# solufast-cvprojects/multigriddet

Hardware: NVIDIA B200
Metric: encode+decode/NMS images/sec, COCO 608×608, 1–8 B200; % HBM peak (higher is better)
Workload: dtype f32

## Files before the change

multigriddet_b200/csrc/api.cu:

```cuda
#include <math.h>
#include <stdarg.h>
#include <stdio.h>
#include <string.h>

#include <chrono>
#include <functional>
#include <mutex>
#include <string>
#include <thread>
#include <vector>

#include "common.cuh"
#include "dlpack_abi.h"

namespace {

thread_local std::string t_error;

int fail(int code, const char* fmt, ...)
{
    char buf[512];
    va_list ap;
    va_start(ap, fmt);
    vsnprintf(buf, sizeof(buf), fmt, ap);
// ... 286 lines not shown

int env_chunk(const char* name)
{
    const char* e = getenv(name);
    return e ? atoi(e) : 0;
}

int chunk_images(const HeadGeom& g, int batch)
{
    long long n = (32ll << 20) / ((long long)g.cells * 4);
    if (const int e = env_chunk("MGD_ENCODE_CHUNK_IMAGES")) n = e;
    if (n < 1) n = 1;
    if (n > batch) n = batch;
    return (int)n;
}

int decode_chunk_images(const HeadGeom& g, int batch)
{
    long long n = (1ll << 30) / ((long long)g.cells * (long long)sizeof(Cand));
    if (const int e = env_chunk("MGD_DECODE_CHUNK_IMAGES")) n = e;
    if (n < 1) n = 1;
    if (n > batch) n = batch;
    return (int)n;
}

struct DeferredStatus {
    int* word[64] = {};
    ~DeferredStatus()
    {
        for (int d = 0; d < 64; ++d) if (word[d]) cudaFree(word[d]);
        cudaGetLastError();
    }
};
thread_local DeferredStatus t_deferred;

int deferred_status_word(int device, int** out)
{
    if (!t_deferred.word[device]) {
        CUDA_TRY(cudaMalloc(reinterpret_cast<void**>(&t_deferred.word[device]), 256));
        CUDA_TRY(cudaMemset(t_deferred.word[device], 0, 256));
    }
    *out = t_deferred.word[device];
    return MGD_OK;
}

int status_to_error(int st)
{
    if (st & 1) return fail(MGD_ERR_CLASS_RANGE, "class id must be less than num_classes");
    if (st & 2)
        return fail(MGD_ERR_INVALID_ARGUMENT,
                    "negative class id on a valid box (the reference would write a wrong channel)");
    return MGD_OK;
}

struct EncodeScratch { int* table; BoxRec* recs; };

bool step_pdl()
{
    static int v = -1;
    if (v < 0) { const char* e = getenv("MGD_STEP_PDL"); v = e ? atoi(e) : 1; }
    return v != 0;
}

int encode_assign_all(const HeadGeom& g, const float* boxes, int batch, int N, float* const* y,
                      cudaStream_t stream, int* d_status, int tf_compat, std::vector<EncodeArgs>* chunks)
{
    nvtx_range nv("mgd:encode assign (preprocess_true_boxes)");
    const Alloc al{nullptr, stream};
    const int step = chunk_images(g, batch);
    for (int b0 = 0; b0 < batch; b0 += step) {
        const int nb = batch - b0 < step ? batch - b0 : step;
        EncodeArgs a;
        a.g = g;
        a.B = nb;
        a.N = N;
        a.boxes = boxes + (size_t)b0 * N * 5;
        for (int l = 0; l < g.L; ++l)
            a.y[l] = y[l] + (size_t)b0 * g.gh[l] * g.gw[l] * g.D[l];
        a.tf_compat = tf_compat;
        a.status = d_status;
        a.stats = nullptr;
        a.big_tables = nullptr;
        a.table = nullptr;
        a.recs = nullptr;
        chunks->push_back(a);
        EncodeArgs& c = chunks->back();
        if (encode_needs_big_tables(g, N))
            CUDA_TRY(al.get(&c.big_tables, (size_t)nb * 2 * g.cells * sizeof(int)));
        CUDA_TRY(al.get(&c.table, (size_t)nb * g.cells * sizeof(int)));
        CUDA_TRY(al.get(&c.recs, (size_t)nb * (N > 0 ? N : 1) * sizeof(BoxRec)));
    }
    struct Group {
        cudaStream_t st;
        explicit Group(cudaStream_t s) : st(s) { prof_group_begin(PROF_ENCODE_ASSIGN, st); }
        ~Group() { prof_group_end(PROF_ENCODE_ASSIGN, st); }
    } group(stream);
    for (size_t k = 0; k < chunks->size(); ++k)
        CUDA_TRY(launch_encode_assign((*chunks)[k], stream, k > 0 && step_pdl()));
    return MGD_OK;
}

int encode_fill_all(std::vector<EncodeArgs>& chunks, int num_sms, cudaStream_t stream)
{
    nvtx_range nv("mgd:encode fill (preprocess_true_boxes)");
    const bool env_pdl = step_pdl();
    bool first = true;
    prof_group_begin(PROF_ENCODE_FILL, stream);
    struct GroupEnd { cudaStream_t st; ~GroupEnd() { prof_group_end(PROF_ENCODE_FILL, st); } } group_end{stream};
    for (EncodeArgs& a : chunks) {
        const cudaError_t e = launch_encode_fill(a, num_sms, stream, env_pdl && !first);
        if (e != cudaSuccess) return fail(MGD_ERR_CUDA, "y_true writer launch failed: %s", cudaGetErrorString(e));
        first = false;
    }
    return MGD_OK;
}

void encode_free_all(std::vector<EncodeArgs>& chunks, cudaStream_t stream)
{
    const Alloc al{nullptr, stream};
    for (EncodeArgs& a : chunks) {
        al.put(a.table); al.put(a.recs); al.put(a.big_tables);
        a.table = nullptr; a.recs = nullptr; a.big_tables = nullptr;
    }
    cudaGetLastError();
}

int encode_device(const HeadGeom& g, const float* boxes, int batch, int N, float* const* y,
                  int num_sms, cudaStream_t stream, int* d_status, unsigned long long* d_stats,
                  const Alloc& al, int tf_compat)
{
    nvtx_range nv("mgd:encode (preprocess_true_boxes)");
    const int step = chunk_images(g, batch);
    for (int b0 = 0; b0 < batch; b0 += step) {
        const int nb = batch - b0 < step ? batch - b0 : step;
        const Arena::Mark mk = al.mark();
        EncodeArgs a;
        a.g = g;
        a.B = nb;
        a.N = N;
        a.boxes = boxes + (size_t)b0 * N * 5;
        for (int l = 0; l < g.L; ++l)
            a.y[l] = y[l] + (size_t)b0 * g.gh[l] * g.gw[l] * g.D[l];
        a.tf_compat = tf_compat;
        a.status = d_status;
        a.stats = d_stats;
        a.big_tables = nullptr;
        if (encode_needs_big_tables(g, N))
            CUDA_TRY(al.get(&a.big_tables, (size_t)nb * 2 * g.cells * sizeof(int)));
        CUDA_TRY(al.get(&a.table, (size_t)nb * g.cells * sizeof(int)));
        CUDA_TRY(al.get(&a.recs, (size_t)nb * (N > 0 ? N : 1) * sizeof(BoxRec)));
        CUDA_TRY(launch_encode(a, num_sms, stream));
        CUDA_TRY(al.put(a.table));
        CUDA_TRY(al.put(a.recs));
        CUDA_TRY(al.put(a.big_tables));
        al.rewind(mk);
    }
    return MGD_OK;
}

}

struct mgd_exchange {
    int device = 0, world = 1, rank = 0;
    size_t bytes = 0;
    char* alloc[MGD_EXCHANGE_MAX_RANKS] = {};
    bool connected = false;
    unsigned epoch = 0;
    cudaIpcMemHandle_t handle;
};

namespace {

std::mutex g_exchange_mutex;
std::vector<mgd_exchange*> g_exchanges;

mgd_exchange* exchange_of(const void* p, int device)
{
    std::lock_guard<std::mutex> lock(g_exchange_mutex);
    const char* c = static_cast<const char*>(p);
    for (mgd_exchange* ex : g_exchanges) {
        const char* lo = ex->alloc[ex->rank] + MGD_EXCHANGE_HEADER_BYTES;
        if (ex->device == device && c >= lo && c < lo + ex->bytes) return ex;
    }
    return nullptr;
}

bool exchange_holds(const mgd_exchange* ex, const void* p, size_t nbytes)
{
    const char* c = static_cast<const char*>(p);
    const char* lo = ex->alloc[ex->rank] + MGD_EXCHANGE_HEADER_BYTES;
    return c >= lo && c + nbytes <= lo + ex->bytes;
}

ExchangeView exchange_view(const mgd_exchange* ex)
{
    ExchangeView v;
    memset(&v, 0, sizeof(v));
    v.world = ex->world;
    v.rank = ex->rank;
    for (int r = 0; r < ex->world; ++r) v.header[r] = reinterpret_cast<unsigned*>(ex->alloc[r]);
    return v;
}

float objectness_prefilter(const mgd_post_config& post)
{
    const double c = post.confidence;
    if (!(c > 0.0)) return -INFINITY;
    if (c >= 1.0) return 15.0f;
    const double logit = log(c / (1.0 - c));
    return (float)(logit - 1e-3 - 1e-4 * fabs(logit));
}

int decode_nms_device(const HeadGeom& g, const mgd_post_config& post, const float* const* preds,
                      int batch, const int* image_hw, double* xywh, int* xyxy, double* scores,
                      int* classes, int* index, int* counts, int num_sms, cudaStream_t stream,
                      unsigned long long* d_stats, const Alloc& al,
                      const std::function<int()>* after_first_decode = nullptr)
{
    nvtx_range nv("mgd:decode+nms (MultiGridDecoder.postprocess)");
    const int step = decode_chunk_images(g, batch);
    const int M = post.max_boxes;
    int pow2 = 2;
    while (pow2 < g.cells) pow2 <<= 1;
    const bool big_sort = g.cells > nms_smem_capacity();
    const bool big_keep = nms_kept_bytes(M) > 64 * 1024;
    int cur_dev = 0;
    CUDA_TRY(cudaGetDevice(&cur_dev));
    mgd_exchange* ex = al.arena ? nullptr : exchange_of(counts, cur_dev);
    if (ex) {
        const struct { const void* p; size_t n; const char* name; } outs[] = {
            {xywh, (size_t)batch * M * 4 * sizeof(double), "boxes_xywh"},
            {xyxy, (size_t)batch * M * 4 * sizeof(int), "boxes_xyxy"},
            {scores, (size_t)batch * M * sizeof(double), "scores"},
            {classes, (size_t)batch * M * sizeof(int), "classes"},
            {index, (size_t)batch * M * sizeof(int), "index"},
// ... 1307 lines not shown
    if (boxes_dtype != MGD_BOXES_I32 && boxes_dtype != MGD_BOXES_F64)
        return fail(MGD_ERR_INVALID_ARGUMENT, "boxes_dtype must be MGD_BOXES_I32 or MGD_BOXES_F64");
    const size_t n = (size_t)batch * max_boxes * 5;
    if (batch > 0 && !params) return fail(MGD_ERR_INVALID_ARGUMENT, "params is NULL");
    if (n > 0 && (!boxes || !out)) return fail(MGD_ERR_INVALID_ARGUMENT, "NULL tensor");
    int num_sms;
    DeviceScope dev_scope;
    if ((rc = prepare_device(device, &num_sms, &dev_scope))) return rc;
    if (batch == 0) return MGD_OK;
    const size_t esz = boxes_dtype == MGD_BOXES_I32 ? 4 : 8;
    BoxOpArgs a;
    memset(&a, 0, sizeof(a));
    a.B = batch; a.N = max_boxes;
    if (memory == MGD_MEM_DEVICE) {
        cudaStream_t st = (cudaStream_t)stream;
        a.in = boxes; a.counts = counts; a.params = params; a.out = out; a.out_f32 = out_f32;
        a.out_counts = out_counts;
        CUDA_TRY(launch_reshape_boxes(a, boxes_dtype == MGD_BOXES_I32, st));
        if (flags & MGD_FLAG_SYNC) CUDA_TRY(cudaStreamSynchronize(st));
        return MGD_OK;
    }
    cudaStream_t* ss;
    if ((rc = host_streams(device, &ss, nullptr))) return rc;
    cudaStream_t st = ss[0];
    const size_t off_out = (n * esz + 7) & ~(size_t)7, off_f32 = off_out + ((n * esz + 7) & ~(size_t)7);
    const size_t off_par = off_f32 + n * 4, off_cnt = off_par + (size_t)batch * 40;
    const size_t off_ocn = off_cnt + (size_t)batch * 4, total = off_ocn + (size_t)batch * 4;
    unsigned char* buf;
    CUDA_TRY(pool_malloc(&buf, total, st));
    if (n) CUDA_TRY(cudaMemcpyAsync(buf, boxes, n * esz, cudaMemcpyHostToDevice, st));
    CUDA_TRY(cudaMemcpyAsync(buf + off_par, params, (size_t)batch * 40, cudaMemcpyHostToDevice, st));
    if (counts) CUDA_TRY(cudaMemcpyAsync(buf + off_cnt, counts, (size_t)batch * 4, cudaMemcpyHostToDevice, st));
    a.in = buf; a.out = buf + off_out; a.out_f32 = reinterpret_cast<float*>(buf + off_f32);
    a.params = reinterpret_cast<const int*>(buf + off_par);
    a.counts = counts ? reinterpret_cast<const int*>(buf + off_cnt) : nullptr;
    a.out_counts = reinterpret_cast<int*>(buf + off_ocn);
    CUDA_TRY(launch_reshape_boxes(a, boxes_dtype == MGD_BOXES_I32, st));
    CUDA_TRY(cudaStreamSynchronize(st));
    if (n) CUDA_TRY(cudaMemcpy(out, buf + off_out, n * esz, cudaMemcpyDeviceToHost));
    if (out_f32 && n) CUDA_TRY(cudaMemcpy(out_f32, buf + off_f32, n * 4, cudaMemcpyDeviceToHost));
    if (out_counts) CUDA_TRY(cudaMemcpy(out_counts, buf + off_ocn, (size_t)batch * 4, cudaMemcpyDeviceToHost));
    CUDA_TRY(cudaFreeAsync(buf, st));
    return MGD_OK;
}

int mgd_encode_ignore_mask(const mgd_head_config* cfg, const float* boxes, int batch, int max_boxes,
                           const float* const* y_pred, float* const* y_true, double ignore_thresh,
                           double eps, float* const* ignore_mask, float* const* assigned_anchor_iou,
                           float* const* max_iou_map, int device, void* stream, int flags)
{
    nvtx_range nv_api("mgd_encode_ignore_mask");
    HeadGeom g;
    int rc = build_geom(cfg, &g);
    if (rc) return rc;
    if (batch < 0 || max_boxes < 0) return fail(MGD_ERR_INVALID_ARGUMENT, "batch and max_boxes must be >= 0");
    if (!y_pred || !ignore_mask || !assigned_anchor_iou || !max_iou_map)
        return fail(MGD_ERR_INVALID_ARGUMENT, "NULL tensor list");
    for (int l = 0; l < g.L && batch > 0; ++l)
        if (!y_pred[l] || !ignore_mask[l] || !assigned_anchor_iou[l] || !max_iou_map[l] || (y_true && !y_true[l]))
            return fail(MGD_ERR_INVALID_ARGUMENT, "NULL tensor for layer %d", l);
    if (!boxes && (long long)batch * max_boxes > 0) return fail(MGD_ERR_INVALID_ARGUMENT, "boxes is NULL");
    if (max_boxes > 65000)
        return fail(MGD_ERR_UNSUPPORTED, "max_boxes per image must be <= 65000, got %d", max_boxes);
    if ((long long)chunk_images(g, batch > 0 ? batch : 1) * max_boxes >= (1ll << 27))
        return fail(MGD_ERR_UNSUPPORTED, "batch chunk x max_boxes too large");
    int num_sms;
    DeviceScope dev_scope;
    if ((rc = prepare_device(device, &num_sms, &dev_scope))) return rc;
    if (batch == 0) return MGD_OK;
    cudaStream_t st = (cudaStream_t)stream;
    int* d_flag;
    if ((rc = deferred_status_word(device, &d_flag))) return rc;
    const Alloc al{nullptr, st};
    const int step = chunk_images(g, batch);
    for (int b0 = 0; b0 < batch; b0 += step) {
        const int nb = batch - b0 < step ? batch - b0 : step;
        EncodeArgs e;
        e.g = g; e.B = nb; e.N = max_boxes;
        e.boxes = boxes + (size_t)b0 * max_boxes * 5;
        for (int l = 0; l < g.L; ++l)
            e.y[l] = y_true ? y_true[l] + (size_t)b0 * g.gh[l] * g.gw[l] * g.D[l] : nullptr;
        e.tf_compat = (flags & MGD_FLAG_TF_COMPAT) != 0;
        e.status = d_flag; e.stats = nullptr;
        e.big_tables = nullptr; e.table = nullptr; e.recs = nullptr;
        unsigned char* scratch = nullptr;
        auto release = [&]() { al.put(e.table); al.put(e.recs); al.put(e.big_tables); al.put(scratch); };
        cudaError_t ce = cudaSuccess;
        if (encode_needs_big_tables(g, max_boxes))
            ce = al.get(&e.big_tables, (size_t)nb * 2 * g.cells * sizeof(int));
        if (ce == cudaSuccess) ce = al.get(&e.table, (size_t)nb * g.cells * sizeof(int));
        if (ce == cudaSuccess) ce = al.get(&e.recs, (size_t)nb * (max_boxes > 0 ? max_boxes : 1) * sizeof(BoxRec));
        const size_t n_gt = (size_t)nb * g.cells * 2;
        const size_t off_area = n_gt * 16, off_cnt = off_area + n_gt * 4;
        if (ce == cudaSuccess) ce = al.get(&scratch, off_cnt + (size_t)nb * g.L * 4);
        if (ce == cudaSuccess) ce = launch_encode_assign(e, st);
        if (ce == cudaSuccess && y_true) ce = launch_encode_fill(e, num_sms, st);
        if (ce == cudaSuccess) {
            LossArgs a;
            memset(&a, 0, sizeof(a));
            a.g = g; a.B = nb; a.ignore_thresh = (float)ignore_thresh; a.eps = (float)eps;
            a.table = e.table; a.recs = e.recs;
            a.gt_boxes = scratch;
            a.gt_area = reinterpret_cast<float*>(scratch + off_area);
            a.gt_count = reinterpret_cast<int*>(scratch + off_cnt);
            for (int l = 0; l < g.L; ++l) {
                const size_t cells_b0 = (size_t)b0 * g.gh[l] * g.gw[l];
                a.y_pred[l] = y_pred[l] + cells_b0 * g.D[l];
                a.ignore[l] = ignore_mask[l] + cells_b0;
                a.assigned[l] = assigned_anchor_iou[l] + cells_b0;
                a.max_iou[l] = max_iou_map[l] + cells_b0;
            }
            ce = launch_ignore_mask(a, st);
        }
        release();
        CUDA_TRY(ce);
    }
    if (flags & MGD_FLAG_SYNC) {
        CUDA_TRY(cudaStreamSynchronize(st));
        return mgd_poll_status(device, stream);
    }
    return MGD_OK;
}

int mgd_letterbox_boxes(const float* boxes, const int* counts, const int* params, int batch,
                        int max_in, int input_h, int input_w, int max_boxes_per_image, int expansion,
                        float* out, int memory, int device, void* stream, int flags)
{
    nvtx_range nv_api("mgd_letterbox_boxes");
    int rc;
    if ((rc = check_memory_arg(memory))) return rc;
    if (batch < 0 || max_in < 0 || max_boxes_per_image < 1)
        return fail(MGD_ERR_INVALID_ARGUMENT, "batch, max_in >= 0 and max_boxes_per_image >= 1 required");
    if (expansion != 1 && expansion != 2 && expansion != 4 && expansion != 8)
        return fail(MGD_ERR_INVALID_ARGUMENT, "expansion must be 1, 2, 4 or 8 (generators.py:2008-2017)");
    if (input_h < 1 || input_w < 1) return fail(MGD_ERR_INVALID_ARGUMENT, "input shape must be positive");
    const long long cap = (long long)max_boxes_per_image * expansion;
    if (cap > (1 << 20)) return fail(MGD_ERR_UNSUPPORTED, "capacity too large");
    if (batch > 0 && (!params || !out || (max_in > 0 && !boxes)))
        return fail(MGD_ERR_INVALID_ARGUMENT, "NULL tensor");
    int num_sms;
    DeviceScope dev_scope;
    if ((rc = prepare_device(device, &num_sms, &dev_scope))) return rc;
    if (batch == 0) return MGD_OK;
    if (memory == MGD_MEM_DEVICE) {
        cudaStream_t st = (cudaStream_t)stream;
        CUDA_TRY(launch_letterbox_boxes(boxes, counts, params, batch, max_in, max_boxes_per_image,
                                        (int)cap, input_h, input_w, out, st));
        if (flags & MGD_FLAG_SYNC) CUDA_TRY(cudaStreamSynchronize(st));
        return MGD_OK;
    }
    cudaStream_t* ss;
    if ((rc = host_streams(device, &ss, nullptr))) return rc;
    cudaStream_t st = ss[0];
    const size_t n_in = (size_t)batch * max_in * 5 * 4, n_out = (size_t)batch * cap * 5 * 4;
    const size_t off_out = (n_in + 15) & ~(size_t)15, off_par = off_out + ((n_out + 15) & ~(size_t)15);
    const size_t off_cnt = off_par + (size_t)batch * 24, total = off_cnt + (size_t)batch * 4;
    unsigned char* buf;
    CUDA_TRY(pool_malloc(&buf, total, st));
    if (n_in) CUDA_TRY(cudaMemcpyAsync(buf, boxes, n_in, cudaMemcpyHostToDevice, st));
    CUDA_TRY(cudaMemcpyAsync(buf + off_par, params, (size_t)batch * 24, cudaMemcpyHostToDevice, st));
    if (counts) CUDA_TRY(cudaMemcpyAsync(buf + off_cnt, counts, (size_t)batch * 4, cudaMemcpyHostToDevice, st));
    cudaError_t e = launch_letterbox_boxes(reinterpret_cast<const float*>(buf),
                                           counts ? reinterpret_cast<const int*>(buf + off_cnt) : nullptr,
                                           reinterpret_cast<const int*>(buf + off_par), batch, max_in,
                                           max_boxes_per_image, (int)cap, input_h, input_w,
                                           reinterpret_cast<float*>(buf + off_out), st);
    if (e == cudaSuccess) e = cudaStreamSynchronize(st);
    if (e == cudaSuccess) e = cudaMemcpy(out, buf + off_out, n_out, cudaMemcpyDeviceToHost);
    cudaFreeAsync(buf, st);
    CUDA_TRY(e);
    return MGD_OK;
}

int mgd_mosaic_merge_boxes(const double* boxes, int num_sources, int max_boxes, const int* params,
                           int batch, int height, int width, double* out, float* out_f32,
                           int* out_counts, int memory, int device, void* stream, int flags)
{
// ... 183 lines not shown
```

multigriddet_b200/csrc/common.cuh:

```cuda
#pragma once
#include <cuda_runtime.h>
#include <stdint.h>
#include "../../include/mgd.h"

#define MGD_MAX_TOTAL_ANCHORS (MGD_MAX_LAYERS * MGD_MAX_ANCHORS_PER_LAYER)

struct HeadGeom {
    int L, C;
    int in_h, in_w;
    int gh[MGD_MAX_LAYERS], gw[MGD_MAX_LAYERS];
    int na[MGD_MAX_LAYERS];
    int D[MGD_MAX_LAYERS];
    int anchor_first[MGD_MAX_LAYERS];
    int K;
    int cell_off[MGD_MAX_LAYERS];
    int cells;
    int anchors_f64;
    float anc32[MGD_MAX_TOTAL_ANCHORS][2];
    double anc64[MGD_MAX_TOTAL_ANCHORS][2];
};

struct __align__(16) BoxRec {
    double fx, fy;
    float tw, th;
    int hot_anchor;
    int hot_class;
};

struct EncodeArgs {
    HeadGeom g;
    int B, N;
    const float* boxes;
    float* y[MGD_MAX_LAYERS];
    int* table;
    int* big_tables;
    BoxRec* recs;
    int tf_compat;
    int* status;
    unsigned long long* stats;
};

struct __align__(16) Cand {
    float score;
    int index;
    float t[4];
    int cls;
    int anchor;
};

struct __align__(16) BoxD { double x, y, w, h; };

struct DecodeArgs {
    HeadGeom g;
    int B;
    const float* pred[MGD_MAX_LAYERS];
    const int* image_hw;
    int use_softmax, rescore;
    double confidence;
    float obj_logit_min;
    float score_lo;
    long long rows_in_layer[MGD_MAX_LAYERS];
    unsigned long long cells_magic[MGD_MAX_LAYERS];
    Cand* cand;
    int* counts;
    int chunk_blocks;
    int debug;
};

#define MGD_MAX_MIRRORS 7
struct NmsArgs {
    HeadGeom g;
    int B;
    int cap;
    const Cand* cand;
    const double* in_boxes;
    const double* in_scores;
    const int* in_classes;
    BoxD* boxes;
    const int* counts;
    const int* image_hw;
    int in_h, in_w;
    double thr;
    int use_diou, per_class, max_boxes;
    int skip_small;
    int soft;
    double soft_sigma, soft_thr;
    double* soft_scratch;
    int wbf;
    int wbf_conf_type;
    const double* in_weights;
    int* wbf_ints;
    int* next_image;
    unsigned long long* sort_scratch;
    int sort_scratch_stride;
    unsigned char* kept_scratch;
    size_t kept_scratch_stride;
    double* out_xywh; int* out_xyxy; double* out_scores; int* out_classes; int* out_index;
    int* out_counts;
    unsigned long long* stats;
    int n_mirrors;
    long long mirror_delta[MGD_MAX_MIRRORS];
    int warp_ctas_per_sm;
};

#define MGD_EXCHANGE_MAX_RANKS 8
#define MGD_EXCHANGE_HEADER_BYTES 512
#define MGD_EXCHANGE_TIMEOUT_WORD 32
struct ExchangeView {
    int world, rank;
    unsigned* header[MGD_EXCHANGE_MAX_RANKS];
};
enum { MGD_EXCHANGE_SIGNAL = 1, MGD_EXCHANGE_WAIT = 2 };
cudaError_t launch_exchange_barrier(const ExchangeView& v, int which, unsigned epoch, int phase,
                                    cudaStream_t stream);

#define MGD_MAX_IOU_THRESHOLDS 16
struct MatchArgs {
    int B, M, N, T;
    const double* det_boxes;
    const double* det_scores;
    const int* det_classes;
    const int* det_counts;
    const double* gt_boxes;
// ... 76 lines not shown
```

multigriddet_b200/csrc/encode.cu:

```cuda
#include <limits.h>
#include <math.h>
#include <string.h>
#include "common.cuh"

namespace {

constexpr int kAssignThreads = 256;
constexpr int kFillThreads = 256;

__device__ __forceinline__ void st_table_keep(int* p, int v)
{
    unsigned long long pol;
    asm volatile("createpolicy.fractional.L2::evict_last.b64 %0, 1.0;" : "=l"(pol));
    asm volatile("st.global.L2::cache_hint.b32 [%0], %1, %2;" ::"l"(p), "r"(v), "l"(pol) : "memory");
}

__device__ __forceinline__ int match_anchor(const HeadGeom& g, float bw, float bh)
{
    int best = 0;
    if (!g.anchors_f64) {
        float top = -INFINITY;
        const float box_area = __fmul_rn(bw, bh);
        for (int i = 0; i < g.K; ++i) {
            const float aw = g.anc32[i][0], ah = g.anc32[i][1];
            const float inter = __fmul_rn(fminf(bw, aw), fminf(bh, ah));
            const float iol = __fdiv_rn(inter, fmaxf(box_area, __fmul_rn(aw, ah)));
            const float r = rintf(__fmul_rn(iol, 1000.0f));
            if (r > top) { top = r; best = i; }
        }
    } else {
        double top = -INFINITY;
        const double box_area = (double)__fmul_rn(bw, bh);
        for (int i = 0; i < g.K; ++i) {
            const double aw = g.anc64[i][0], ah = g.anc64[i][1];
            const double inter = __dmul_rn(fmin((double)bw, aw), fmin((double)bh, ah));
            const double iol = __ddiv_rn(inter, fmax(box_area, __dmul_rn(aw, ah)));
            const double r = rint(__dmul_rn(iol, 1000.0));
            if (r > top) { top = r; best = i; }
        }
    }
    return best;
}

__device__ __forceinline__ int match_anchor_tf(const HeadGeom& g, float bw, float bh)
{
    int best = 0;
    float top = -INFINITY;
    const float box_area = __fmul_rn(bw, bh);
    for (int i = 0; i < g.K; ++i) {
        const float aw = g.anc32[i][0], ah = g.anc32[i][1];
        const float inter = __fmul_rn(fminf(bw, aw), fminf(bh, ah));
        const float iol = __fdiv_rn(inter, __fadd_rn(fmaxf(box_area, __fmul_rn(aw, ah)), 1e-7f));
        if (iol > top) { top = iol; best = i; }
    }
    return best;
}

__device__ __forceinline__ int pack_place(int layer, int col, int row)
{
    col = min(max(col, -2), 16380) + 2;
    row = min(max(row, -2), 16380) + 2;
    return (layer << 28) | (row << 14) | col;
}

__global__ void __launch_bounds__(kAssignThreads)
encode_assign_kernel(const __grid_constant__ EncodeArgs a)
{
    extern __shared__ int sm[];
    asm volatile("griddepcontrol.launch_dependents;" ::: "memory");
    const HeadGeom& g = a.g;
    const bool big = a.big_tables != nullptr;
    int* cover = big ? a.big_tables + (size_t)blockIdx.x * 2 * g.cells : sm;
    int* owner = cover + g.cells;
    int* place = big ? sm : owner + g.cells;
    __shared__ unsigned int s_stat[3];
    __shared__ int s_status;

    const int b = blockIdx.x;
    const int tid = threadIdx.x;
    for (int i = tid; i < g.cells; i += kAssignThreads) { cover[i] = INT_MAX; owner[i] = -1; }
    if (tid < 3) s_stat[tid] = 0;
    if (tid == 0) s_status = 0;
    __syncthreads();

    unsigned int n_valid = 0, n_skipped = 0, n_pos = 0;
    int status = 0;

    if (a.tf_compat) {
        for (int t = tid; t < a.N; t += kAssignThreads) {
            const float* bx = a.boxes + ((size_t)b * a.N + t) * 5;
            const float x1 = bx[0], y1 = bx[1], x2 = bx[2], y2 = bx[3], cf = bx[4];
            const float bw = __fsub_rn(x2, x1), bh = __fsub_rn(y2, y1);
            if (!(__fmul_rn(bw, bh) > 0.0f)) continue;
            ++n_valid;
            const float cxp = __fmul_rn(__fadd_rn(x1, x2), 0.5f);
            const float cyp = __fmul_rn(__fadd_rn(y1, y2), 0.5f);
            const int ga = match_anchor_tf(g, bw, bh);
// ... 27 lines not shown
                }
            }
        }
        __syncthreads();
    } else {
        for (int t = tid; t < a.N; t += kAssignThreads) {
            const float* bx = a.boxes + ((size_t)b * a.N + t) * 5;
            const float x1 = bx[0], y1 = bx[1], x2 = bx[2], y2 = bx[3], cf = bx[4];
            if (!(cf < (float)g.C)) status |= 1;
            const float bw = __fsub_rn(x2, x1), bh = __fsub_rn(y2, y1);
            int pl = -1;
            if (!(__fmul_rn(bw, bh) <= 0.0f)) {
                ++n_valid;
                const int cls = (int)cf;
                if (cls < 0) status |= 2;
                const float cxp = floorf(__fmul_rn(__fadd_rn(x1, x2), 0.5f));
                const float cyp = floorf(__fmul_rn(__fadd_rn(y1, y2), 0.5f));
                const int ga = match_anchor(g, bw, bh);
                int layer = 0;
                while (layer + 1 < g.L && ga >= g.anchor_first[layer + 1]) ++layer;
                const int k = ga - g.anchor_first[layer];
                const double gx = __dmul_rn((double)cxp, __ddiv_rn((double)g.gh[layer], (double)g.in_h));
                const double gy = __dmul_rn((double)cyp, __ddiv_rn((double)g.gw[layer], (double)g.in_w));
                const int col = (int)fmin(fmax(gx, -4.0), 1.0e6);
                const int row = (int)fmin(fmax(gy, -4.0), 1.0e6);
                BoxRec rec;
                rec.fx = __dsub_rn(gx, (double)col);
                rec.fy = __dsub_rn(gy, (double)row);
                if (!g.anchors_f64) {
                    const float rw = __fdiv_rn(bw, g.anc32[ga][0]);
                    const float rh = __fdiv_rn(bh, g.anc32[ga][1]);
                    rec.tw = (float)log(rw < 1e-3f ? 1e-3 : (double)rw);
                    rec.th = (float)log(rh < 1e-3f ? 1e-3 : (double)rh);
                } else {
                    const double rw = __ddiv_rn((double)bw, g.anc64[ga][0]);
                    const double rh = __ddiv_rn((double)bh, g.anc64[ga][1]);
                    rec.tw = (float)log(rw < 1e-3 ? 1e-3 : rw);
                    rec.th = (float)log(rh < 1e-3 ? 1e-3 : rh);
                }
                rec.hot_anchor = 5 + k;
                rec.hot_class = 5 + g.na[layer] + max(cls, 0);
                a.recs[(size_t)b * a.N + t] = rec;
                pl = pack_place(layer, col, row);
                const int g0 = g.gh[layer], g1 = g.gw[layer];
                const int c0 = (pl & 0x3fff) - 2, r0 = ((pl >> 14) & 0x3fff) - 2;
                #pragma unroll
                for (int dx = -1; dx <= 1; ++dx) {
                    #pragma unroll
                    for (int dy = -1; dy <= 1; ++dy) {
                        const int cc = c0 + dx, rr = r0 + dy;
                        if (cc >= 0 && cc < g0 && rr >= 0 && rr < g1)
                            atomicMin(&cover[g.cell_off[layer] + rr * g1 + cc], t);
                    }
                }
            }
            place[t] = pl;
        }
        __syncthreads();

        for (int t = tid; t < a.N; t += kAssignThreads) {
            const int pl = place[t];
            if (pl < 0) continue;
            const int layer = pl >> 28;
            const int c0 = (pl & 0x3fff) - 2, r0 = ((pl >> 14) & 0x3fff) - 2;
            const int g0 = g.gh[layer], g1 = g.gw[layer];
            int written = 0;
            #pragma unroll
            for (int dx = -1; dx <= 1; ++dx) {
                #pragma unroll
                for (int dy = -1; dy <= 1; ++dy) {
                    const int cc = c0 + dx, rr = r0 + dy;
                    if (cc < 0 || cc >= g0 || rr < 0 || rr >= g1) continue;
                    const int cell = g.cell_off[layer] + rr * g1 + cc;
                    if (cover[cell] < t && written >= 3) { ++n_skipped; continue; }
                    ++written;
                    atomicMax(&owner[cell], t * 16 + (dx + 1) * 3 + (dy + 1));
                }
            }
        }
        __syncthreads();
    }

    const int rec_base = b * a.N * 16;
    for (int l = 0; l < g.L; ++l) {
        const int n = g.gh[l] * g.gw[l];
        int* dst = a.table + (size_t)a.B * g.cell_off[l] + (size_t)b * n;
        const int* src = owner + g.cell_off[l];
        for (int i = tid; i < n; i += kAssignThreads) {
            const int v = src[i];
            st_table_keep(dst + i, v < 0 ? -1 : v + rec_base);
            n_pos += (v >= 0);
        }
    }
    if (n_valid) atomicAdd(&s_stat[0], n_valid);
    if (n_skipped) atomicAdd(&s_stat[1], n_skipped);
    if (n_pos) atomicAdd(&s_stat[2], n_pos);
    if (status) atomicOr(&s_status, status);
    __syncthreads();
    if (tid < 3 && a.stats && s_stat[tid]) atomicAdd(&a.stats[tid], (unsigned long long)s_stat[tid]);
    if (tid == 0 && s_status) atomicOr(a.status, s_status);
}

struct FillPlan {
    int dv[MGD_MAX_LAYERS];
    int R[MGD_MAX_LAYERS];
    long long tile_first[MGD_MAX_LAYERS + 1];
    long long rows[MGD_MAX_LAYERS];
    int debug;
};

template <int VEC> struct VecT;
template <> struct VecT<4> { using type = float4; };
template <> struct VecT<1> { using type = float; };

__device__ __forceinline__ unsigned nth_bit(unsigned m, int n)
{
    #pragma unroll
    for (int q = 0; q < 3; ++q)
        if (q < n) m &= m - 1;
    return m ? (unsigned)(__ffs((int)m) - 1) : 32u;
}

template <int VEC>
__global__ void __launch_bounds__(kFillThreads)
encode_fill_kernel(const __grid_constant__ EncodeArgs a, const __grid_constant__ FillPlan p)
{
    using V = typename VecT<VEC>::type;
    asm volatile("griddepcontrol.launch_dependents;" ::: "memory");
    const HeadGeom& g = a.g;
    const int lane = threadIdx.x & 31;
    const long long warp = ((long long)blockIdx.x * kFillThreads + threadIdx.x) >> 5;
    const long long n_warps = ((long long)gridDim.x * kFillThreads) >> 5;
    const long long total = p.tile_first[g.L];
    V zero;
    if constexpr (VEC == 4) zero = make_float4(0.f, 0.f, 0.f, 0.f); else zero = 0.f;

    auto tile_layer = [&](long long tile) {
        int l = 0;
        while (l + 1 < g.L && tile >= p.tile_first[l + 1]) ++l;
        return l;
    };
    auto load_codes = [&](long long tile) {
        if (tile >= total || (p.debug & 1)) return -1;
        const int l = tile_layer(tile);
        const long long row = (tile - p.tile_first[l]) * p.R[l] + lane;
        if (lane >= p.R[l] || row >= p.rows[l]) return -1;
        return __ldg(a.table + (size_t)a.B * g.cell_off[l] + row);
    };

    int next_codes = load_codes(warp);
    for (long long tile = warp; tile < total; tile += n_warps) {
        const int codes = next_codes;
        next_codes = load_codes(tile + n_warps);
        const int l = tile_layer(tile);
        const int dv = p.dv[l];
        const long long row0 = (tile - p.tile_first[l]) * p.R[l];
        const long long left = p.rows[l] - row0;
        const int n_rows = (int)(left < p.R[l] ? left : p.R[l]);
        const int n_units = n_rows * dv;

        V* dst = reinterpret_cast<V*>(a.y[l]) + row0 * dv;
        #pragma unroll 4
        for (int f = lane; f < n_units; f += 32) dst[f] = zero;

        unsigned pos = __ballot_sync(0xffffffffu, codes >= 0);
        if (pos) {
            __syncwarp();
            const int slot = lane >> 3, role = lane & 7;
            float* ybase = a.y[l] + row0 * (long long)g.D[l];
            while (pos) {
                const unsigned r = nth_bit(pos, slot);
                const int code = __shfl_sync(0xffffffffu, codes, r & 31);
                if (r < 32u && role < 7) {
                    const BoxRec* rec = a.recs + (code >> 4);
                    const int nb = code & 15;
                    int ch = role;
                    float v = 1.0f;
                    if (role == 0)      v = (float)__dadd_rn((double)(1 - nb / 3), rec->fx);
                    else if (role == 1) v = (float)__dadd_rn((double)(1 - nb % 3), rec->fy);
                    else if (role == 2) v = rec->tw;
                    else if (role == 3) v = rec->th;
                    else if (role == 5) ch = rec->hot_anchor;
                    else if (role == 6) ch = rec->hot_class;
                    ybase[(long long)r * g.D[l] + ch] = v;
                }
                #pragma unroll
                for (int q = 0; q < 4; ++q) pos &= pos - 1;
            }
        }
    }
}

}

size_t encode_assign_smem_bytes(const HeadGeom& g, int N)
{
    return (size_t)(2 * g.cells + N) * sizeof(int);
}

bool encode_needs_big_tables(const HeadGeom& g, int N)
{
    return encode_assign_smem_bytes(g, N) > 200 * 1024;
}

cudaError_t launch_encode(const EncodeArgs& a, int num_sms, cudaStream_t stream)
{
    cudaError_t err = launch_encode_assign(a, stream);
    if (err != cudaSuccess) return err;
    return launch_encode_fill(a, num_sms, stream);
}

cudaError_t launch_encode_assign(const EncodeArgs& a, cudaStream_t stream, bool overlap_previous)
{
    const HeadGeom& g = a.g;
    const size_t smem = a.big_tables ? (size_t)a.N * sizeof(int) + 16 : encode_assign_smem_bytes(g, a.N);
    cudaError_t err = cudaFuncSetAttribute(encode_assign_kernel,
                                           cudaFuncAttributeMaxDynamicSharedMemorySize, (int)smem);
    if (err != cudaSuccess) return err;
    prof_mark_begin(PROF_ENCODE_ASSIGN, stream);
    if (overlap_previous) {
        cudaLaunchConfig_t cfg;
        memset(&cfg, 0, sizeof(cfg));
        cfg.gridDim = dim3((unsigned)a.B);
        cfg.blockDim = dim3(kAssignThreads);
        cfg.dynamicSmemBytes = smem;
        cfg.stream = stream;
        cudaLaunchAttribute attr;
        attr.id = cudaLaunchAttributeProgrammaticStreamSerialization;
        attr.val.programmaticStreamSerializationAllowed = 1;
        cfg.attrs = &attr;
        cfg.numAttrs = 1;
        const cudaError_t e = cudaLaunchKernelEx(&cfg, encode_assign_kernel, a);
        prof_mark_end(PROF_ENCODE_ASSIGN, stream);
        return e != cudaSuccess ? e : cudaGetLastError();
    }
    encode_assign_kernel<<<a.B, kAssignThreads, smem, stream>>>(a);
    prof_mark_end(PROF_ENCODE_ASSIGN, stream);
    return cudaGetLastError();
}

cudaError_t launch_encode_fill(const EncodeArgs& a, int num_sms, cudaStream_t stream, bool overlap_previous)
{
    const HeadGeom& g = a.g;
    bool vec4 = true;
    for (int l = 0; l < g.L; ++l)
        vec4 = vec4 && (g.D[l] % 4 == 0) && ((reinterpret_cast<uintptr_t>(a.y[l]) & 15) == 0);
    const int vec = vec4 ? 4 : 1;
    FillPlan p;
    long long tiles = 0;
    for (int l = 0; l < g.L; ++l) {
        p.dv[l] = g.D[l] / vec;
        int gcd = p.dv[l], t = 32;
        while (t) { const int m = gcd % t; gcd = t; t = m; }
        p.R[l] = 32 / gcd;
        p.rows[l] = (long long)a.B * g.gh[l] * g.gw[l];
        p.tile_first[l] = tiles;
        tiles += (p.rows[l] + p.R[l] - 1) / p.R[l];
    }
    p.tile_first[g.L] = tiles;
    static int env_dbg = -1;
    if (env_dbg < 0) { const char* e = getenv("MGD_FILL_DEBUG"); env_dbg = e ? atoi(e) : 0; }
    p.debug = env_dbg;
    long long blocks = (tiles * 32 + kFillThreads - 1) / kFillThreads;
    static int env_waves = -1;
    if (env_waves < 0) { const char* e = getenv("MGD_FILL_MAX_WAVES"); env_waves = e ? atoi(e) : 0; }
    if (env_waves > 0) {
        const long long max_blocks = (long long)num_sms * (2048 / kFillThreads) * env_waves;
        if (blocks > max_blocks) blocks = max_blocks;
    }
    if (blocks > 0x7fffffffll) blocks = 0x7fffffffll;
    if (blocks < 1) blocks = 1;
    prof_mark_begin(PROF_ENCODE_FILL, stream);
    if (overlap_previous) {
        cudaLaunchConfig_t cfg;
        memset(&cfg, 0, sizeof(cfg));
        cfg.gridDim = dim3((unsigned)blocks);
        cfg.blockDim = dim3(kFillThreads);
        cfg.stream = stream;
        cudaLaunchAttribute attr;
        attr.id = cudaLaunchAttributeProgrammaticStreamSerialization;
        attr.val.programmaticStreamSerializationAllowed = 1;
        cfg.attrs = &attr;
        cfg.numAttrs = 1;
        const cudaError_t e = vec4 ? cudaLaunchKernelEx(&cfg, encode_fill_kernel<4>, a, p)
                                   : cudaLaunchKernelEx(&cfg, encode_fill_kernel<1>, a, p);
        prof_mark_end(PROF_ENCODE_FILL, stream);
        return e != cudaSuccess ? e : cudaGetLastError();
    }
    if (vec4) encode_fill_kernel<4><<<(unsigned)blocks, kFillThreads, 0, stream>>>(a, p);
    else      encode_fill_kernel<1><<<(unsigned)blocks, kFillThreads, 0, stream>>>(a, p);
    prof_mark_end(PROF_ENCODE_FILL, stream);
    return cudaGetLastError();
}
```

Measured before the change: 1.394 million.

## Add per-cell occupancy bitmap so y_true fill skips dense owner-table reads

New measurement: 1.401 million, median of 6. Within noise of the previous version (+0.5%).

```diff
diff --git a/multigriddet_b200/csrc/api.cu b/multigriddet_b200/csrc/api.cu
--- a/multigriddet_b200/csrc/api.cu
+++ b/multigriddet_b200/csrc/api.cu
@@ -392,6 +392,7 @@
         a.stats = nullptr;
         a.big_tables = nullptr;
         a.table = nullptr;
+        a.bitmap = nullptr;
         a.recs = nullptr;
         chunks->push_back(a);
         EncodeArgs& c = chunks->back();
@@ -400,11 +401,17 @@
         CUDA_TRY(al.get(&c.table, (size_t)nb * g.cells * sizeof(int)));
         CUDA_TRY(al.get(&c.recs, (size_t)nb * (N > 0 ? N : 1) * sizeof(BoxRec)));
     }
+    long long words = 0;
+    for (const EncodeArgs& c : *chunks) words += encode_bitmap_word(g, c.B, g.L);
+    unsigned* bitmap = nullptr;
+    CUDA_TRY(al.get(&bitmap, (size_t)words * sizeof(unsigned)));
+    for (EncodeArgs& c : *chunks) { c.bitmap = bitmap; bitmap += encode_bitmap_word(g, c.B, g.L); }
     struct Group {
         cudaStream_t st;
         explicit Group(cudaStream_t s) : st(s) { prof_group_begin(PROF_ENCODE_ASSIGN, st); }
         ~Group() { prof_group_end(PROF_ENCODE_ASSIGN, st); }
     } group(stream);
+    CUDA_TRY(cudaMemsetAsync(chunks->front().bitmap, 0, (size_t)words * sizeof(unsigned), stream));
     for (size_t k = 0; k < chunks->size(); ++k)
         CUDA_TRY(launch_encode_assign((*chunks)[k], stream, k > 0 && step_pdl()));
     return MGD_OK;
@@ -428,9 +435,10 @@
 void encode_free_all(std::vector<EncodeArgs>& chunks, cudaStream_t stream)
 {
     const Alloc al{nullptr, stream};
+    if (!chunks.empty()) al.put(chunks.front().bitmap);
     for (EncodeArgs& a : chunks) {
         al.put(a.table); al.put(a.recs); al.put(a.big_tables);
-        a.table = nullptr; a.recs = nullptr; a.big_tables = nullptr;
+        a.table = nullptr; a.recs = nullptr; a.big_tables = nullptr; a.bitmap = nullptr;
     }
     cudaGetLastError();
 }
@@ -458,9 +466,13 @@
         if (encode_needs_big_tables(g, N))
             CUDA_TRY(al.get(&a.big_tables, (size_t)nb * 2 * g.cells * sizeof(int)));
         CUDA_TRY(al.get(&a.table, (size_t)nb * g.cells * sizeof(int)));
+        const size_t bitmap_bytes = (size_t)encode_bitmap_word(g, nb, g.L) * sizeof(unsigned);
+        CUDA_TRY(al.get(&a.bitmap, bitmap_bytes));
         CUDA_TRY(al.get(&a.recs, (size_t)nb * (N > 0 ? N : 1) * sizeof(BoxRec)));
+        CUDA_TRY(cudaMemsetAsync(a.bitmap, 0, bitmap_bytes, stream));
         CUDA_TRY(launch_encode(a, num_sms, stream));
         CUDA_TRY(al.put(a.table));
+        CUDA_TRY(al.put(a.bitmap));
         CUDA_TRY(al.put(a.recs));
         CUDA_TRY(al.put(a.big_tables));
         al.rewind(mk);
@@ -1934,17 +1946,20 @@
             e.y[l] = y_true ? y_true[l] + (size_t)b0 * g.gh[l] * g.gw[l] * g.D[l] : nullptr;
         e.tf_compat = (flags & MGD_FLAG_TF_COMPAT) != 0;
         e.status = d_flag; e.stats = nullptr;
-        e.big_tables = nullptr; e.table = nullptr; e.recs = nullptr;
+        e.big_tables = nullptr; e.table = nullptr; e.bitmap = nullptr; e.recs = nullptr;
         unsigned char* scratch = nullptr;
-        auto release = [&]() { al.put(e.table); al.put(e.recs); al.put(e.big_tables); al.put(scratch); };
+        auto release = [&]() { al.put(e.table); al.put(e.bitmap); al.put(e.recs); al.put(e.big_tables); al.put(scratch); };
         cudaError_t ce = cudaSuccess;
         if (encode_needs_big_tables(g, max_boxes))
             ce = al.get(&e.big_tables, (size_t)nb * 2 * g.cells * sizeof(int));
         if (ce == cudaSuccess) ce = al.get(&e.table, (size_t)nb * g.cells * sizeof(int));
+        const size_t bitmap_bytes = (size_t)encode_bitmap_word(g, nb, g.L) * sizeof(unsigned);
+        if (ce == cudaSuccess) ce = al.get(&e.bitmap, bitmap_bytes);
         if (ce == cudaSuccess) ce = al.get(&e.recs, (size_t)nb * (max_boxes > 0 ? max_boxes : 1) * sizeof(BoxRec));
         const size_t n_gt = (size_t)nb * g.cells * 2;
         const size_t off_area = n_gt * 16, off_cnt = off_area + n_gt * 4;
         if (ce == cudaSuccess) ce = al.get(&scratch, off_cnt + (size_t)nb * g.L * 4);
+        if (ce == cudaSuccess) ce = cudaMemsetAsync(e.bitmap, 0, bitmap_bytes, st);
         if (ce == cudaSuccess) ce = launch_encode_assign(e, st);
         if (ce == cudaSuccess && y_true) ce = launch_encode_fill(e, num_sms, st);
         if (ce == cudaSuccess) {
diff --git a/multigriddet_b200/csrc/common.cuh b/multigriddet_b200/csrc/common.cuh
--- a/multigriddet_b200/csrc/common.cuh
+++ b/multigriddet_b200/csrc/common.cuh
@@ -33,12 +33,20 @@
     const float* boxes;
     float* y[MGD_MAX_LAYERS];
     int* table;
+    unsigned* bitmap;
     int* big_tables;
     BoxRec* recs;
     int tf_compat;
     int* status;
     unsigned long long* stats;
 };
+
+__host__ __device__ inline long long encode_bitmap_word(const HeadGeom& g, int B, int l)
+{
+    long long w = 0;
+    for (int k = 0; k < l; ++k) w += ((long long)B * g.gh[k] * g.gw[k] + 31) >> 5;
+    return w;
+}
 
 struct __align__(16) Cand {
     float score;
diff --git a/multigriddet_b200/csrc/encode.cu b/multigriddet_b200/csrc/encode.cu
--- a/multigriddet_b200/csrc/encode.cu
+++ b/multigriddet_b200/csrc/encode.cu
@@ -13,6 +13,13 @@
     unsigned long long pol;
     asm volatile("createpolicy.fractional.L2::evict_last.b64 %0, 1.0;" : "=l"(pol));
     asm volatile("st.global.L2::cache_hint.b32 [%0], %1, %2;" ::"l"(p), "r"(v), "l"(pol) : "memory");
+}
+
+__device__ __forceinline__ void red_or_keep(unsigned* p, unsigned v)
+{
+    unsigned long long pol;
+    asm volatile("createpolicy.fractional.L2::evict_last.b64 %0, 1.0;" : "=l"(pol));
+    asm volatile("red.global.or.L2::cache_hint.b32 [%0], %1, %2;" ::"l"(p), "r"(v), "l"(pol) : "memory");
 }
 
 __device__ __forceinline__ int match_anchor(const HeadGeom& g, float bw, float bh)
@@ -206,14 +213,23 @@
     }
 
     const int rec_base = b * a.N * 16;
+    const int lane = tid & 31;
     for (int l = 0; l < g.L; ++l) {
         const int n = g.gh[l] * g.gw[l];
         int* dst = a.table + (size_t)a.B * g.cell_off[l] + (size_t)b * n;
+        unsigned* bits = a.bitmap + encode_bitmap_word(g, a.B, l);
         const int* src = owner + g.cell_off[l];
-        for (int i = tid; i < n; i += kAssignThreads) {
-            const int v = src[i];
-            st_table_keep(dst + i, v < 0 ? -1 : v + rec_base);
+        for (int i = tid; i - lane < n; i += kAssignThreads) {
+            const int v = i < n ? src[i] : -1;
+            if (i < n) st_table_keep(dst + i, v < 0 ? -1 : v + rec_base);
             n_pos += (v >= 0);
+            const unsigned m = __ballot_sync(0xffffffffu, v >= 0);
+            if (m) {
+                const long long r = (long long)b * n + (i - lane);
+                const int s = (int)(r & 31);
+                const unsigned part = lane == 0 ? m << s : (s ? m >> (32 - s) : 0u);
+                if (lane < 2 && part) red_or_keep(bits + (r >> 5) + lane, part);
+            }
         }
     }
     if (n_valid) atomicAdd(&s_stat[0], n_valid);
@@ -230,6 +246,7 @@
     int R[MGD_MAX_LAYERS];
     long long tile_first[MGD_MAX_LAYERS + 1];
     long long rows[MGD_MAX_LAYERS];
+    long long word_first[MGD_MAX_LAYERS];
     int debug;
 };
 
@@ -264,18 +281,18 @@
         while (l + 1 < g.L && tile >= p.tile_first[l + 1]) ++l;
         return l;
     };
-    auto load_codes = [&](long long tile) {
-        if (tile >= total || (p.debug & 1)) return -1;
+    auto load_mask = [&](long long tile) -> unsigned {
+        if (tile >= total || (p.debug & 1)) return 0u;
         const int l = tile_layer(tile);
-        const long long row = (tile - p.tile_first[l]) * p.R[l] + lane;
-        if (lane >= p.R[l] || row >= p.rows[l]) return -1;
-        return __ldg(a.table + (size_t)a.B * g.cell_off[l] + row);
+        const long long row0 = (tile - p.tile_first[l]) * p.R[l];
+        const unsigned w = __ldg(a.bitmap + p.word_first[l] + (row0 >> 5));
+        return (w >> (row0 & 31)) & (0xffffffffu >> (32 - p.R[l]));
     };
 
-    int next_codes = load_codes(warp);
+    unsigned next_mask = load_mask(warp);
     for (long long tile = warp; tile < total; tile += n_warps) {
-        const int codes = next_codes;
-        next_codes = load_codes(tile + n_warps);
+        const unsigned mask = next_mask;
+        next_mask = load_mask(tile + n_warps);
         const int l = tile_layer(tile);
         const int dv = p.dv[l];
         const long long row0 = (tile - p.tile_first[l]) * p.R[l];
@@ -287,8 +304,10 @@
         #pragma unroll 4
         for (int f = lane; f < n_units; f += 32) dst[f] = zero;
 
-        unsigned pos = __ballot_sync(0xffffffffu, codes >= 0);
+        unsigned pos = mask;
         if (pos) {
+            const int codes = (pos >> lane) & 1u
+                ? __ldg(a.table + (size_t)a.B * g.cell_off[l] + row0 + lane) : -1;
             __syncwarp();
             const int slot = lane >> 3, role = lane & 7;
             float* ybase = a.y[l] + row0 * (long long)g.D[l];
@@ -379,6 +398,7 @@
         p.R[l] = 32 / gcd;
         p.rows[l] = (long long)a.B * g.gh[l] * g.gw[l];
         p.tile_first[l] = tiles;
+        p.word_first[l] = encode_bitmap_word(g, a.B, l);
         tiles += (p.rows[l] + p.R[l] - 1) / p.R[l];
     }
     p.tile_first[g.L] = tiles;
```
